# zbqq/neus2

Hardware: AMD Instinct MI355X
Metric: training samples/sec (compacted NeuS2 training samples, DTU-scan24-shaped synthetic, base.json) (higher is better)
Workload: dtype fp16 MFMA (fp32 accumulate) / fp32 optimizer; 1 GPU; NeuS2 train step, Config S, base.json L=14 T=2^19 W=64, Nc=2^18/GPU, R=2^18/GPU fixed, all 14 levels active (network trained 800 steps before the warm-up); global_batch=262144, rays_per_gpu=262144, parallelism=dp1, prepare_steps=800, levels_active=14

## Files before the change

include/neus2_hip.h:

```cpp
#ifndef NEUS2_HIP_H
#define NEUS2_HIP_H

#include <stdint.h>

#ifdef __cplusplus
extern "C" {
#endif

typedef struct NeusTestbed NeusTestbed;

typedef struct NeusNetworkConfig {
	uint32_t n_levels;
	uint32_t n_features_per_level;
	uint32_t log2_hashmap_size;
	uint32_t base_resolution;
	float per_level_scale;
	float top_resolution;
	float valid_level_scale;
	float base_valid_level_scale;
	uint32_t base_training_step;
	uint32_t n_neurons;
	uint32_t n_density_hidden;
	uint32_t n_rgb_hidden;
	float learning_rate, beta1, beta2, epsilon, l2_reg;
// ... 135 lines not shown
	float background_color[3];
	int32_t color_space;
	int32_t linear_colors;
	float cone_angle_constant;
	float near_distance;
	float depth_supervision_lambda;
} NeusTrainingOptions;
int neus_testbed_get_training_options(NeusTestbed* tb, NeusTrainingOptions* out);
typedef struct NeusOptimizerState {
	uint32_t n_params;
	uint32_t current_step;
	float learning_rate;
	float learning_rate_factor;
} NeusOptimizerState;
int neus_testbed_get_optimizer_state(NeusTestbed* tb, NeusOptimizerState* st, float* m1, float* m2, uint32_t* steps, uint16_t* ema_half);
int neus_testbed_set_optimizer_state(NeusTestbed* tb, const NeusOptimizerState* st, const float* m1, const float* m2, const uint32_t* steps,
                                     const uint16_t* ema_half);
int neus_testbed_set_training_options(NeusTestbed* tb, const NeusTrainingOptions* opts);
int neus_testbed_set_progressive_inference(NeusTestbed* tb, int mode, const uint32_t* chunk_ends, uint32_t n_ends);
int neus_testbed_ray_counts(NeusTestbed* tb, uint32_t n, uint32_t* nreq, uint32_t* ccount, uint32_t* numsteps );
int neus_debug_time_kernel(NeusTestbed* tb, int kernel, int variant, int iters, float* ms_out);
int neus_testbed_time_kernel(NeusTestbed* tb, int kernel, int iters, float* ms_out, uint32_t* units_out);
int neus_debug_march_stats(NeusTestbed* tb, uint32_t n, uint32_t* out);
int neus_debug_march_profile(NeusTestbed* tb, unsigned long long* out, uint32_t max_waves, uint32_t* n_waves);
int neus_debug_scatter_stats(NeusTestbed* tb, uint64_t* records_per_level, uint32_t* max_region);
int neus_debug_scatter_parts(NeusTestbed* tb, uint32_t* parts_per_level );
int neus_debug_grid_scatter(NeusTestbed* tb, void* hip_stream, uint32_t n_cap, const uint32_t* n_valid, const float* coords,
                            uint32_t coord_stride, uint32_t valid_level, const void* dLdenc, const void* genc, const float* v,
                            float* grid_grad_out);
int neus_debug_mlp_train(NeusTestbed* tb, void* hip_stream, uint32_t n, const float* coords, const uint16_t* enc, const float* dydx,
                         const uint16_t* dL_dout, uint32_t indeed_batch_size, float* grads_out, float* dpos, uint16_t* genc_out,
                         uint16_t* dLdenc_out, uint16_t* d1_delta_out, float* v_out);
int neus_debug_exclusive_scan(void* hip_stream, const uint32_t* in, uint32_t* out, uint32_t n, int reps, uint32_t* failures);
int neus_debug_scan_giveup(void* hip_stream, const uint32_t* in, uint32_t* out, uint32_t n, uint32_t* failures);
int neus_debug_inject_health(NeusTestbed* tb, uint32_t flags);
int neus_debug_set_lds_fill(NeusTestbed* tb, uint32_t pattern);
int neus_debug_set_lds_fill_all(NeusTestbed* tb, uint32_t pattern);
int neus_debug_set_xcd_shift(NeusTestbed* tb, uint32_t n_blocks);
int neus_debug_set_grid_generic(uint32_t on);
int neus_debug_get_batch(NeusTestbed* tb, float* coords_out, uint16_t* dl_dout_out, float* loss_out);
int neus_debug_denorm_probe(int device, uint32_t n, uint32_t launches, uint64_t* stats);
int neus_debug_get_buffer(NeusTestbed* tb, int id, uint64_t offset, uint64_t nbytes, void* host);
int neus_debug_replay_loss_grad(NeusTestbed* tb, uint16_t* dl_dout_out);
int neus_debug_sample_rays_round0(NeusTestbed* tb, void* stream, uint32_t n_rays, uint32_t n_rays_total, uint64_t rng_state, uint64_t rng_inc,
                                  uint32_t max_samples, const uint8_t* bitfield, float* rays, uint32_t* numsteps, float* coords,
                                  uint32_t* counters_out, uint32_t chunk_end, uint32_t* list, uint32_t* list_len, uint32_t lds_fill);
int neus_testbed_stream(NeusTestbed* tb, void** hip_stream);
int neus_testbed_synchronize(NeusTestbed* tb);
#define NEUS_N_PHASES 10
int neus_testbed_set_profiling(NeusTestbed* tb, int on);
int neus_testbed_kernel_times(NeusTestbed* tb, float* ms_out );
int neus_testbed_set_infer_timing(NeusTestbed* tb, int on);
int neus_testbed_infer_timing(NeusTestbed* tb, double* ms_total, uint64_t* launches, uint64_t* steps);
int neus_testbed_set_exchange_timing(NeusTestbed* tb, int on);
int neus_testbed_exchange_timing(NeusTestbed* tb, double* exposed_ms_total, double* span_ms_total, uint64_t* steps);

int neus_nccl_unique_id(uint8_t* out );
int neus_testbed_init_data_parallel(NeusTestbed* tb, int rank, int world, const uint8_t* unique_id );
#define NEUS_DP_FORCE_COLLECTIVES 1
int neus_testbed_init_data_parallel_ex(NeusTestbed* tb, int rank, int world, const uint8_t* unique_id, uint32_t flags);
typedef struct NeusDataParallelInfo {
	uint32_t rank, world;
	uint32_t has_communicator;
	uint32_t local_group;
	uint64_t collective_calls;
	uint64_t allreduce_bytes;
// ... 93 lines not shown
```

neus2_amd/_lib.py:

```python
from __future__ import annotations

import ctypes as C
import os

_HERE = os.path.dirname(os.path.abspath(__file__))
LIB_PATH = os.environ.get("NEUS2_HIP_LIB") or os.path.join(_HERE, "libneus2_hip.so")


class NeusNetworkConfig(C.Structure):
    _fields_ = [
        ("n_levels", C.c_uint32), ("n_features_per_level", C.c_uint32), ("log2_hashmap_size", C.c_uint32),
        ("base_resolution", C.c_uint32), ("per_level_scale", C.c_float), ("top_resolution", C.c_float),
        ("valid_level_scale", C.c_float), ("base_valid_level_scale", C.c_float), ("base_training_step", C.c_uint32),
        ("n_neurons", C.c_uint32), ("n_density_hidden", C.c_uint32), ("n_rgb_hidden", C.c_uint32),
        ("learning_rate", C.c_float), ("beta1", C.c_float), ("beta2", C.c_float), ("epsilon", C.c_float), ("l2_reg", C.c_float),
        ("ema_decay", C.c_float), ("decay_start", C.c_uint32), ("decay_interval", C.c_uint32), ("decay_base", C.c_float),
        ("ek_loss_weight", C.c_float), ("mask_loss_weight", C.c_float), ("anneal_end", C.c_uint32), ("batch_size", C.c_uint32),
        ("sdf_bias", C.c_float), ("density_grid_decay", C.c_float), ("seed", C.c_uint32), ("fixed_rays_per_batch", C.c_uint32),
        ("predict_global_movement", C.c_uint32), ("global_movement_steps", C.c_uint32), ("finetune_global_movement", C.c_uint32),
        ("reset_density_grid_after_global_movement", C.c_uint32), ("after_learning_rate", C.c_float),
        ("gm_learning_rate", C.c_float), ("gm_beta1", C.c_float), ("gm_beta2", C.c_float), ("gm_epsilon", C.c_float),
        ("gm_decay_start", C.c_uint32), ("gm_decay_interval", C.c_uint32), ("gm_decay_base", C.c_float),
    ]

# ... 50 lines not shown
        ("width", C.c_int32), ("height", C.c_int32), ("spp", C.c_uint32), ("training_view", C.c_int32),
        ("xform", C.c_float * 12), ("focal", C.c_float * 2), ("screen_center", C.c_float * 2),
        ("snap_to_pixel_centers", C.c_int32), ("min_transmittance", C.c_float), ("use_ema", C.c_int32),
    ]


class NeusTrainingOptions(C.Structure):
    _fields_ = [
        ("random_bg_color", C.c_int32), ("background_color", C.c_float * 3), ("color_space", C.c_int32),
        ("linear_colors", C.c_int32), ("cone_angle_constant", C.c_float), ("near_distance", C.c_float),
        ("depth_supervision_lambda", C.c_float),
    ]


class NeusOptimizerState(C.Structure):
    _fields_ = [("n_params", C.c_uint32), ("current_step", C.c_uint32), ("learning_rate", C.c_float),
                ("learning_rate_factor", C.c_float)]


class NeusModuleInfo(C.Structure):
    _fields_ = [("n_params", C.c_uint64), ("n_input_dims", C.c_uint32), ("n_output_dims", C.c_uint32),
                ("param_precision", C.c_int32), ("output_precision", C.c_int32), ("gradient_precision", C.c_int32),
                ("batch_capacity", C.c_uint32), ("n_levels", C.c_uint32), ("grid_offset", C.c_uint64),
                ("per_level_scale", C.c_float)]


EXPORTS = [
    "neus_last_error", "neus_abi_version", "neus_device_count", "neus_device_synchronize",
    "neus_testbed_create", "neus_testbed_destroy", "neus_testbed_set_dataset", "neus_testbed_reload_network",
    "neus_testbed_layout", "neus_testbed_train", "neus_testbed_get_stats", "neus_testbed_get_params",
    "neus_testbed_set_params", "neus_testbed_get_gradients", "neus_testbed_get_ema_params",
    "neus_testbed_get_half_params",
    "neus_testbed_get_density_grid", "neus_testbed_set_density_grid", "neus_testbed_restore_state", "neus_testbed_get_rng", "neus_testbed_render", "neus_testbed_sdf_on_grid",
    "neus_testbed_marching_cubes", "neus_testbed_mc_density", "neus_testbed_get_mesh", "neus_testbed_mesh_vertex_colors", "neus_mc_table", "neus_prepare_image_rgba8", "neus_testbed_ray_counts", "neus_debug_time_kernel", "neus_debug_march_stats", "neus_debug_exclusive_scan", "neus_debug_scan_giveup", "neus_debug_inject_health", "neus_debug_set_lds_fill", "neus_debug_set_lds_fill_all", "neus_debug_set_xcd_shift", "neus_debug_set_grid_generic", "neus_debug_denorm_probe", "neus_debug_get_batch", "neus_debug_get_buffer", "neus_debug_replay_loss_grad", "neus_debug_sample_rays_round0", "neus_debug_march_profile", "neus_debug_scatter_stats", "neus_debug_scatter_parts", "neus_debug_grid_scatter", "neus_debug_mlp_train", "neus_testbed_time_kernel", "neus_testbed_stream",
    "neus_testbed_synchronize", "neus_testbed_set_profiling", "neus_testbed_kernel_times", "neus_testbed_set_infer_timing", "neus_testbed_infer_timing",
    "neus_testbed_set_exchange_timing", "neus_testbed_exchange_timing",
    "neus_nccl_unique_id", "neus_testbed_init_data_parallel", "neus_testbed_init_data_parallel_ex",
    "neus_testbed_data_parallel_info", "neus_testbed_set_exchange_overlap", "neus_local_group_create", "neus_local_group_destroy",
    "neus_testbed_init_local_group", "neus_host_group_create", "neus_host_group_destroy", "neus_testbed_init_host_group", "neus_debug_host_group_allreduce",
    "neus_grid_encode", "neus_net_forward", "neus_net_backward", "neus_sample_rays", "neus_loss_compact",
    "neus_optimizer_step", "neus_fill_rollover", "neus_occ_update", "neus_mfma_probe",
    "neus_testbed_next_frame", "neus_testbed_get_movement", "neus_testbed_set_movement", "neus_testbed_frame_state",
    "neus_testbed_change_frame", "neus_testbed_prepare_for_test", "neus_testbed_get_training_options",
    "neus_testbed_set_training_options", "neus_testbed_saved_transform", "neus_testbed_get_optimizer_state",
    "neus_testbed_set_optimizer_state", "neus_testbed_set_progressive_inference",
    "neus_module_create_network", "neus_module_create_nerf_network", "neus_module_create_encoding", "neus_module_create_network_with_input_encoding", "neus_module_destroy", "neus_context_destroy",
    "neus_module_info", "neus_module_hyperparams", "neus_module_set_training_step", "neus_module_set_indeed_batch_size",
    "neus_module_initialize_params", "neus_module_inference", "neus_module_forward", "neus_module_backward",
    "neus_module_backward_backward_input",
    "neus_net_backward_pos", "neus_delta_apply", "neus_delta_backward",
    "neus_volrend_march_count", "neus_volrend_march_write", "neus_volrend_alpha_forward", "neus_volrend_alpha_backward",
    "neus_volrend_composite_forward", "neus_volrend_composite_backward",
]

ABI_VERSION = 9

_lib = None


def lib():
    global _lib
    if _lib is not None:
        return _lib
    if not os.path.exists(LIB_PATH):
        raise RuntimeError(f"{LIB_PATH} not found: build it with `python -c 'import __graft_entry__ as g; g.build()'`")
    l = C.CDLL(LIB_PATH)
    l.neus_last_error.restype = C.c_char_p
# ... 21 lines not shown
```

neus2_amd/csrc/kernels.h:

```cpp
#pragma once
#include <functional>
#include <vector>
#include "common.h"

namespace neus {

struct MlpPtrs {
	const half_t* d0;  const half_t* d1;
	const half_t* r0;  const half_t* r1;  const half_t* r2;
	const half_t* d0T; const half_t* d1T;
	const half_t* r0T; const half_t* r1T; const half_t* r2T;
	const half_t* d0p; const half_t* d0Tp;
	const half_t* var;
	float sdf_bias;
};

struct TrainBufs {
	half_t* d1_delta;
	half_t* dLdenc; half_t* genc;
	float4* v;
	float* var_grad;
	float* var_partial;
	float indeed_batch;
	float4* dpos;
// ... 242 lines not shown
uint32_t ray_sort_blocks(uint32_t cap);
void launch_ray_sort(hipStream_t s, uint32_t cap, const uint32_t* numsteps, const float* coords, uint32_t e1, const RaySort& rs, uint32_t* list,
                     uint32_t* list_len, void* scan_temp, size_t scan_temp_bytes, const RaySplit* split = nullptr);
void launch_march_write(hipStream_t s, uint32_t cap, StepState* st, const DevDataset& ds, const float* rays, const MarchWork& mw, const uint32_t* nreq,
                        uint32_t* base, uint32_t* numsteps, float* coords, uint32_t* sample_ray, uint32_t sample_cap, void* scan_temp,
                        const Round0List* round0 = nullptr, uint32_t lds_fill = 0 );
constexpr uint32_t FILL_LDS_BYTES = 40 * 1024;
void launch_fill_lds(hipStream_t s, uint32_t pattern);
extern thread_local uint32_t g_dbg_lds_fill;
extern thread_local uint32_t g_dbg_xcd_shift;
extern thread_local hipEvent_t g_infer_ev[2];
void debug_denorm_probe(hipStream_t s, uint32_t n, uint32_t launches, uint64_t* stats);
void launch_xcd_shift(hipStream_t s, uint32_t n_blocks);
inline void dbg_lds_gate(hipStream_t s) {
	if (g_dbg_lds_fill) launch_fill_lds(s, g_dbg_lds_fill);
	if (g_dbg_xcd_shift) launch_xcd_shift(s, g_dbg_xcd_shift);
}
void debug_launch_march_stats(hipStream_t s, uint32_t n_rays, const float* rays, const float* tstart, const uint32_t* lin, const DevDataset& ds,
                              const uint8_t* bf, uint32_t* out);
void launch_loss_alpha(hipStream_t s, uint32_t cap_samples, const StepState* st, const float* coords, const half_t* net_out, float cos_anneal,
                       const LossWork& w, bool dt_const = false);
void launch_loss_scan_ray(hipStream_t s, uint32_t cap_rays, const uint32_t* numsteps, const LossWork& w, uint32_t* ccount);
void launch_loss_alpha_list(hipStream_t s, uint32_t cap_samples, const uint32_t* n_ptr, const uint32_t* idx, const float* coords,
                            const half_t* net_out, float cos_anneal, const LossWork& w, bool dt_const = false);
void launch_prog_cut(hipStream_t s, uint32_t cap_rays, const uint32_t* ccount, const uint32_t* excl, uint32_t batch, uint32_t* cutw, int mode,
                     uint32_t* eval0, uint32_t* abort_if_none = nullptr);
void launch_scan_prog_cut(hipStream_t s, void* scan_temp, const uint32_t* ccount, uint32_t* excl, uint32_t n, uint32_t batch, uint32_t* cutw, int mode,
                          uint32_t* eval0, uint32_t* abort_if_none = nullptr);
void launch_prog_next(hipStream_t s, uint32_t cap_rays, const uint32_t* rays_in, const uint32_t* n_in, const uint32_t* numsteps, const uint32_t* cut,
                      uint32_t e1, uint32_t e2, uint32_t* list, uint32_t* list_counter, uint32_t* rays_out, uint32_t* n_out);
void launch_loss_scan_chunk(hipStream_t s, uint32_t cap_rays, const uint32_t* numsteps, const LossWork& w, uint32_t* ccount, uint32_t e0,
                            uint32_t e1, uint32_t e2, uint32_t* list , uint32_t* next_counter,
                            const uint32_t* rays_in = nullptr, const uint32_t* n_rays_in = nullptr, uint32_t* rays_out = nullptr,
                            uint32_t* n_rays_out = nullptr);
void launch_srgb_lut(hipStream_t s, float* lut);
void launch_loss_ray(hipStream_t s, uint32_t cap_rays, StepState* st, DPInfo dp, const DevDataset& ds, const LossParams& lp, uint32_t* numsteps,
                     const uint32_t* ccount, const uint32_t* cbase, const LossWork& w, float* loss, float* ek, float* mask);
void launch_loss_grad(hipStream_t s, uint32_t cap_samples, StepState* st, DPInfo dp, const LossParams& lp, const float* coords,
                      const half_t* net_out, const uint32_t* numsteps, const LossWork& w, float* coords_out, half_t* dL_dout);
void debug_launch_loss_scan(hipStream_t s, int variant, uint32_t cap_rays, const uint32_t* numsteps, const LossWork& w, uint32_t* ccount);
void launch_ray_index(hipStream_t s, uint32_t cap_rays, const uint32_t* numsteps, StepState* st, uint32_t* sample_ray, uint32_t* rbase);
void launch_rollover(hipStream_t s, uint32_t n_elements, const StepState* st, float* coords, half_t* dL_dout);
void launch_step_counters(hipStream_t s, StepState* st, uint32_t target_batch, uint32_t max_samples, uint32_t world, uint32_t fixed_rays,
                          const uint32_t* eval_cnt = nullptr, uint32_t n_eval = 0, uint32_t* abort_host = nullptr);
size_t render_ray_bytes();
void launch_render_init(hipStream_t s, const RenderCamera& cam, uint32_t sample_index, const DevDataset& ds, const uint8_t* bf, const uint32_t* lin,
                        void* rays, float4* frame);
void launch_render_compact(hipStream_t s, uint32_t n, const void* src, uint32_t* flags, uint32_t* base, void* dst, uint32_t* n_alive,
                           void* scan_tmp, size_t scan_tmp_bytes);
void launch_render_gen(hipStream_t s, uint32_t n_alive, uint32_t n_steps, const DevDataset& ds, const uint8_t* bf, const uint32_t* lin, void* rays,
                       float* coords);
void launch_render_composite(hipStream_t s, uint32_t n_alive, uint32_t n_steps, const float* coords, const half_t* net_out, float cos_anneal,
                             float min_transmittance, bool linear_colors, void* rays, float4* frame);
void launch_render_accumulate(hipStream_t s, uint32_t n, uint32_t spp, const float4* frame, float4* accum);
uint32_t mc_n_chunks(const uint32_t res[3]);
void mc_table_host(int8_t* out );
void launch_mc_count(hipStream_t s, const uint32_t res[3], const float amin[3], const float amax[3], float thresh, const float* density,
                     uint32_t* cnt_v, uint32_t* cnt_t);
void launch_mc_emit(hipStream_t s, const uint32_t res[3], const float amin[3], const float amax[3], float thresh, const float* density,
                    const uint32_t* off_v, const uint32_t* off_t, float* verts, uint32_t* vidx, uint32_t* tris);
void launch_mesh_coords(hipStream_t s, uint32_t n, const float* verts, const DevDataset& ds, float* coords);
void launch_mesh_unmove(hipStream_t s, uint32_t n, const RayMotion& m, float* verts);
void launch_delta_prepare(hipStream_t s, DeltaState* ds);
void launch_delta_apply(hipStream_t s, const uint32_t* n_ptr, uint32_t n_cap, uint32_t stride, const float* in, float* out, const DeltaState* ds);
void launch_delta_backward(hipStream_t s, const uint32_t* n_ptr, uint32_t n_cap, const float* coords, uint32_t stride, const float4* dpos,
                           DeltaState* ds, float* partial, const DeltaAdam& a);
void launch_delta_grad(hipStream_t s, const uint32_t* n_ptr, uint32_t n_cap, const float* coords, uint32_t stride, const float4* dpos,
// ... 86 lines not shown
```

neus2_amd/csrc/march.hip:

```cpp
#pragma clang fp contract(off)
#include "march_common.h"
#include "scan_lookback.h"
#include <algorithm>
#include <cstdlib>
#include <cstring>
#include <vector>

namespace neus {



__global__ void k_bitfield_linear(const uint8_t* __restrict__ bf, uint32_t* __restrict__ lin) {
	const uint32_t w = blockIdx.x * blockDim.x + threadIdx.x;
	if (w >= GRID3 / 32) return;
	const uint32_t ix = w >> 9, iy = (w >> 2) & 127, iz0 = (w & 3) * 32;
	uint32_t word = 0;
	for (uint32_t b = 0; b < 32; ++b) {
		const uint32_t idx = morton3D(ix, iy, iz0 + b);
		word |= (uint32_t)((bf[idx / 8] >> (idx % 8)) & 1) << b;
	}
	lin[w] = word;
}
__device__ __forceinline__ bool ray_hits_box(const float o[3], const float d[3], const float bb[6]) {
	float tn = 0.0f, tf = 3.402823466e+38f;
// ... 1120 lines not shown
			}
		}
		if (open) {
			ccount[i] = S.cn;
			racc[i] = make_float4(S.r0, S.r1, S.r2, S.ws);
			rT[i] = S.T;
			rek[i] = S.ek;
		}
		if (list || rays_out) {
			const uint32_t m = (open && S.cn == e1 && e1 < ns && S.T >= 1e-4f) ? min(ns, e2) - e1 : 0u;
			const uint32_t incl = wave_incl_sum(m);
			const uint32_t total = wave_lane_value(incl, 63);
			if (total) {
				if (list) {
					uint32_t p0 = 0;
					if (lane == 0) p0 = atomicAdd(next_counter, total);
					p0 = wave_lane_value(p0, 0);
					const uint32_t pre = incl - m, src = base + e1;
					unsigned long long todo = __ballot(m > 0);
					while (todo) {
						const int o = __ffsll(todo) - 1;
						todo &= todo - 1ull;
						const uint32_t m_o = wave_lane_value(m, o), p_o = p0 + wave_lane_value(pre, o), s_o = wave_lane_value(src, o);
						for (uint32_t j = lane; j < m_o; j += 64) list[p_o + j] = s_o + j;
					}
				}
				if (rays_out) {
					const unsigned long long mk = __ballot(m > 0);
					uint32_t q0 = 0;
					if (lane == 0) q0 = atomicAdd(n_rays_out, (uint32_t)__popcll(mk));
					q0 = wave_lane_value(q0, 0);
					if (m > 0) rays_out[q0 + (uint32_t)__popcll(mk & ((1ull << lane) - 1ull))] = i;
				}
			}
		}
	}
}

__global__ void __launch_bounds__(256) k_prog_cut(uint32_t cap_rays, const uint32_t* __restrict__ ccount, const uint32_t* __restrict__ excl,
                                                  uint32_t batch, uint32_t* __restrict__ cutw, int mode, uint32_t* __restrict__ eval0,
                                                  uint32_t* __restrict__ abort_if_none) {
	const uint32_t i = blockIdx.x * blockDim.x + threadIdx.x;
	if (i >= cap_rays) return;
	const uint32_t e = excl[i], incl = e + ccount[i];
	const bool cross = e < batch && incl >= batch, none = i == cap_rays - 1 && incl < batch;
	if (!cross && !none) return;
	const uint32_t c = cross ? i : cap_rays;
	if (mode == 0) {
		cutw[CW_CUT_A] = c;
		cutw[CW_LENB_EFF] = cross ? 0u : cutw[CW_LENB];
		cutw[CW_NB_EFF] = cross ? 0u : cutw[CW_NB];
	} else {
		cutw[CW_CUT] = c;
		cutw[CW_EST] = min(cap_rays, (c + c / 4u + 1024u + 63u) & ~63u);
		if (eval0) *eval0 += cutw[CW_LENB_EFF];
		if (abort_if_none && !cross) *abort_if_none = 1u;
	}
}
__global__ void __launch_bounds__(SCAN_THREADS) k_scan_prog_cut(const uint32_t* __restrict__ ccount, uint32_t* __restrict__ excl, uint32_t n,
                                                                ScanState* __restrict__ ss, uint32_t tag, uint32_t batch, uint32_t* __restrict__ cutw,
                                                                int mode, uint32_t* __restrict__ eval0, uint32_t* __restrict__ abort_if_none) {
	__shared__ uint32_t s_prefix, s_wsum[SCAN_THREADS / 64];
	const ScanTile tl = scan_tile(tag);
	const size_t b0 = (size_t)tl.tile * SCAN_TILE + (size_t)threadIdx.x * SCAN_ITEMS;
	uint32_t v[SCAN_ITEMS];
	scan_load16(ccount, b0, n, true, v);
// ... 397 lines not shown
void launch_march_write(hipStream_t s, uint32_t cap, StepState* st, const DevDataset& ds, const float* rays, const MarchWork& mw, const uint32_t* nreq,
                        uint32_t* base, uint32_t* numsteps, float* coords, uint32_t* sample_ray, uint32_t sample_cap, void* scan_temp,
                        const Round0List* round0, uint32_t lds_fill) {
	const Round0List r0 = round0 ? *round0 : Round0List{0u, nullptr, nullptr, nullptr, 0u};
	if (cap % 4 || ((uintptr_t)nreq | (uintptr_t)base | (uintptr_t)numsteps | (uintptr_t)r0.c0) & 15)
		throw std::runtime_error("launch_march_write: ray buffers must be 16-B aligned, cap a multiple of 4");
	const uint32_t tiles = (cap + SCAN_TILE - 1) / SCAN_TILE;
	if (tiles > SCAN_MAX_TILES) throw std::runtime_error("launch_march_write: too many ray slots");
	dbg_lds_gate(s);
	k_march_scan<<<tiles, SCAN_THREADS, 0, s>>>(cap, st, nreq, base, numsteps, (ScanState*)scan_temp, scan_next_tag(scan_temp), r0);
	if (lds_fill) launch_fill_lds(s, lds_fill);
	else dbg_lds_gate(s);
	k_march_write<<<std::max<uint32_t>(1, (sample_cap + WRITE_CHUNK - 1) / WRITE_CHUNK), 256, 0, s>>>(cap, st, ds, rays, mw, nreq, base, coords, sample_ray,
	                                                                                                      r0);
}
void debug_launch_march_stats(hipStream_t s, uint32_t n_rays, const float* rays, const float* tstart, const uint32_t* lin, const DevDataset& ds,
                              const uint8_t* bf, uint32_t* out) {
	k_march_stats<<<(n_rays + 255) / 256, 256, 0, s>>>(n_rays, rays, tstart, lin, ds, bf, out);
}
static inline uint32_t sample_blocks(uint32_t cap) { return std::max<uint32_t>(1, std::min<uint32_t>((cap + 255) / 256, 16384)); }
void launch_loss_alpha(hipStream_t s, uint32_t cap_samples, const StepState* st, const float* coords, const half_t* net_out, float cos_anneal,
                       const LossWork& w, bool dt_const) {
	dbg_lds_gate(s);
	k_loss_alpha<<<sample_blocks(cap_samples), 256, 0, s>>>(cap_samples, &st->n_kept, nullptr, coords, net_out, cos_anneal, w.sa, w.ekt, w.n_long,
	                                                        dt_const);
}
void launch_loss_alpha_list(hipStream_t s, uint32_t cap_samples, const uint32_t* n_ptr, const uint32_t* idx, const float* coords,
                            const half_t* net_out, float cos_anneal, const LossWork& w, bool dt_const) {
	dbg_lds_gate(s);
	k_loss_alpha<<<sample_blocks(cap_samples), 256, 0, s>>>(cap_samples, n_ptr, idx, coords, net_out, cos_anneal, w.sa, w.ekt, nullptr, dt_const);
}
void launch_loss_scan_chunk(hipStream_t s, uint32_t cap_rays, const uint32_t* numsteps, const LossWork& w, uint32_t* ccount, uint32_t e0,
                            uint32_t e1, uint32_t e2, uint32_t* list, uint32_t* next_counter, const uint32_t* rays_in, const uint32_t* n_rays_in,
                            uint32_t* rays_out, uint32_t* n_rays_out) {
	dbg_lds_gate(s);
	k_loss_scan_chunk<<<std::max<uint32_t>(1, std::min<uint32_t>((cap_rays + 63) / 64, 8192)), 64, 0, s>>>(
		cap_rays, numsteps, w.sa, w.ekt, w.ck4, w.cke, ccount, w.racc, w.rT, w.rek, e0, e1, e2, list, next_counter, rays_in, n_rays_in,
		rays_out, n_rays_out);
}
void launch_prog_cut(hipStream_t s, uint32_t cap_rays, const uint32_t* ccount, const uint32_t* excl, uint32_t batch, uint32_t* cutw, int mode,
                     uint32_t* eval0, uint32_t* abort_if_none) {
	k_prog_cut<<<(cap_rays + 255) / 256, 256, 0, s>>>(cap_rays, ccount, excl, batch, cutw, mode, eval0, abort_if_none);
}
void launch_prog_next(hipStream_t s, uint32_t cap_rays, const uint32_t* rays_in, const uint32_t* n_in, const uint32_t* numsteps, const uint32_t* cut,
                      uint32_t e1, uint32_t e2, uint32_t* list, uint32_t* list_counter, uint32_t* rays_out, uint32_t* n_out) {
	k_prog_next<<<std::max<uint32_t>(1, std::min<uint32_t>((cap_rays + 255) / 256, 1024)), 256, 0, s>>>(rays_in, n_in, numsteps, cut, e1, e2, list,
	                                                                                                   list_counter, rays_out, n_out);
}
void launch_loss_scan_ray(hipStream_t s, uint32_t cap_rays, const uint32_t* numsteps, const LossWork& w, uint32_t* ccount) {
	const uint32_t blocks = ray_blocks(cap_rays);
	dbg_lds_gate(s);
	k_loss_scan_ray<true><<<blocks, 256, 0, s>>>(cap_rays, numsteps, w.sa, w.ekt, w.ck4, w.cke, ccount, w.racc, w.rT, w.long_rays, w.n_long);
	if (w.long_rays) dbg_lds_gate(s);
	if (w.long_rays) k_loss_scan_list<<<std::max<uint32_t>(1, std::min<uint32_t>((cap_rays + 63) / 64, 4096)), 64, 0, s>>>(
		numsteps, w.sa, w.ekt, w.ck4, w.cke, ccount, w.racc, w.rT, w.long_rays, w.n_long);
}
void debug_launch_loss_scan(hipStream_t s, int variant, uint32_t cap_rays, const uint32_t* numsteps, const LossWork& w, uint32_t* ccount) {
	if (variant == 1) k_loss_scan_ray<false><<<ray_blocks(cap_rays), 256, 0, s>>>(cap_rays, numsteps, w.sa, w.ekt, w.ck4, w.cke, ccount, w.racc, w.rT,
	                                                                           nullptr, nullptr);
	else {
		if (w.n_long) (void)hipMemsetAsync(w.n_long, 0, 4, s);
		launch_loss_scan_ray(s, cap_rays, numsteps, w, ccount);
	}
}
__global__ void k_srgb_lut(float* __restrict__ lut) {
	const uint32_t b = threadIdx.x;
	lut[b] = srgb_to_linear((float)b * (1.0f / 255.0f));
}
// ... 29 lines not shown
```

neus2_amd/csrc/options.h:

```cpp
#pragma once

#include <algorithm>
#include <cstdint>
#include <cstdio>
#include <cstdlib>
#include <cstring>
#include <vector>

namespace neus_env {
inline bool on_unless_0(const char* name) { const char* e = std::getenv(name); return !(e && e[0] == '0'); }
inline bool off_unless_1(const char* name) { const char* e = std::getenv(name); return e && e[0] == '1'; }
inline bool is(const char* name, const char* value) { const char* e = std::getenv(name); return e && std::strcmp(e, value) == 0; }
inline int as_int(const char* name, int def) { const char* e = std::getenv(name); return e ? std::atoi(e) : def; }
inline uint32_t as_u32(const char* name, uint32_t def) { const char* e = std::getenv(name); return e ? (uint32_t)std::strtoul(e, nullptr, 10) : def; }
inline float as_float(const char* name, float def) { const char* e = std::getenv(name); return e ? (float)std::atof(e) : def; }
inline std::vector<uint32_t> increasing_list(const char* name) {
	std::vector<uint32_t> v;
	const char* e = std::getenv(name);
	if (!e) return v;
	for (const char* p = e; *p;) { char* q = nullptr; const unsigned long x = std::strtoul(p, &q, 10); if (q == p) break; v.push_back((uint32_t)x); p = *q ? q + 1 : q; }
	bool ok = !v.empty() && v.size() <= 14 && v[0] > 0;
	for (size_t k = 1; k < v.size(); ++k) ok = ok && v[k] > v[k - 1];
	if (!ok) v.clear();
	return v;
}
}

struct NeusOptions {
	bool main_prio = true;
	bool lookahead = true;
	int la_at_cut = 1;
	int la_at_full = 0;
	int la_prio = -1;
	bool ev_sysfence = false;
	bool la_stat = false;
	bool adam_overlap = false;
	bool exchange_overlap = true;
	bool eager_ema_h = false;

	uint32_t march_waves = 0;
	uint32_t march_lanes = 8;
	bool march_balance = true;
	uint32_t march_dbg = 0;
	bool ray_cull = true;
	bool ray_sort = true;
	bool prog_cut = true;
	bool march_cut = true;
	uint32_t march_cut_div = 1;
	std::vector<uint32_t> chunk_ends;
	float chunk_scale = 2.f;
	int chunk_rounds = 2;

	bool occ_sort = true;
	bool occ_nu_sort = false;

	uint32_t scatter_mode = 2;
	uint32_t scatter_chunk = 512;
	uint32_t scatter_level_groups = 0;
	uint32_t scatter_xcd_group = 4;
	bool scatter_noskip = false;

	bool dbg_loss_replay = false;
	bool dbg_loss_fence = false;

	static NeusOptions from_env() {
		using namespace neus_env;
		NeusOptions o;
		o.main_prio = on_unless_0("NEUS_MAIN_PRIO");
		o.lookahead = on_unless_0("NEUS_LOOKAHEAD");
		o.la_at_cut = as_int("NEUS_LA_AT", o.la_at_cut);
		o.la_at_full = as_int("NEUS_LA_AT_FULL", o.la_at_full);
		o.la_prio = as_int("NEUS_LA_PRIO", o.la_prio);
		o.ev_sysfence = off_unless_1("NEUS_EV_SYSFENCE");
		o.la_stat = off_unless_1("NEUS_LA_STAT");
		o.adam_overlap = off_unless_1("NEUS_ADAM_OVERLAP");
		o.exchange_overlap = on_unless_0("NEUS_EXCHANGE_OVERLAP");
		o.eager_ema_h = off_unless_1("NEUS_EAGER_EMA_H");
		o.march_waves = as_u32("NEUS_MARCH_WAVES", o.march_waves);
		{ const uint32_t v = as_u32("NEUS_MARCH_LANES", 8); o.march_lanes = v == 1 || v == 4 || v == 16 ? v : 8u; }
		o.march_balance = on_unless_0("NEUS_MARCH_BALANCE");
		o.march_dbg = as_u32("NEUS_MARCH_DBG", o.march_dbg);
		o.ray_cull = on_unless_0("NEUS_RAY_CULL");
		o.ray_sort = on_unless_0("NEUS_RAY_SORT");
		o.prog_cut = on_unless_0("NEUS_PROG_CUT");
		o.march_cut = on_unless_0("NEUS_MARCH_CUT");
		o.march_cut_div = (uint32_t)std::max(1, as_int("NEUS_DBG_MARCH_CUT_DIV", 1));
		o.chunk_ends = increasing_list("NEUS_CHUNK_ENDS");
		o.chunk_scale = as_float("NEUS_CHUNK_SCALE", o.chunk_scale);
		o.chunk_rounds = as_int("NEUS_CHUNK_ROUNDS", o.chunk_rounds);
		o.occ_sort = on_unless_0("NEUS_OCC_SORT");
		o.occ_nu_sort = off_unless_1("NEUS_OCC_NU_SORT");
		o.scatter_mode = is("NEUS_SCATTER", "binned") ? 1u : is("NEUS_SCATTER", "wide") ? 0u : 2u;
		o.scatter_chunk = is("NEUS_SCATTER_CHUNK", "1024") ? 1024u : is("NEUS_SCATTER_CHUNK", "256") ? 256u : 512u;
		if (o.scatter_mode != 2 && o.scatter_chunk == 256) o.scatter_chunk = 512;
		o.scatter_level_groups = (uint32_t)std::max(0, as_int("NEUS_SCATTER_LG", 0));
		o.scatter_xcd_group = std::max(1u, as_u32("NEUS_SC_XCD_GROUP", o.scatter_xcd_group));
		o.scatter_noskip = off_unless_1("NEUS_SCATTER_NOSKIP");
		o.dbg_loss_replay = off_unless_1("NEUS_DBG_LOSS_REPLAY");
		o.dbg_loss_fence = off_unless_1("NEUS_DBG_LOSS_FENCE");
		return o;
	}
};

struct NeusProcessOptions {
	bool infer_xcd_parts = false;
	bool infer_pipe = true;
	uint32_t infer_grid = 0;
	uint32_t mlp_blocks_pct = 100;
	static NeusProcessOptions from_env() {
		using namespace neus_env;
		NeusProcessOptions o;
		o.infer_xcd_parts = off_unless_1("NEUS_INFER_XCD_PARTS");
		o.infer_pipe = on_unless_0("NEUS_INFER_PIPE");
		o.infer_grid = (uint32_t)as_int("NEUS_INFER_GRID", 0);
		o.mlp_blocks_pct = (uint32_t)as_int("NEUS_MLP_BLOCKS_PCT", 100);
		return o;
	}
};
inline const NeusProcessOptions& process_options() {
	static const NeusProcessOptions o = NeusProcessOptions::from_env();
	return o;
}
// ... 14 lines not shown
```

neus2_amd/csrc/testbed.cpp:

```cpp
#include <rocprofiler-sdk-roctx/roctx.h>
#include "kernels.h"
#include "scan_lookback.h"
#include "json_lite.h"
#include "hostgroup.h"
#include "options.h"
#include "host_util.h"
#include "core.h"
#include "../../include/neus2_hip.h"

#include <rccl/rccl.h>

#include <algorithm>
#include <atomic>
#include <cstdio>
#include <functional>
#include <chrono>
#include <cmath>
#include <condition_variable>
#include <mutex>
#include <cstdlib>
#include <cstring>
#include <memory>
#include <random>
#include <stdexcept>
// ... 1383 lines not shown
		const bool sorted_rays = progressive && opt.ray_sort;
		const RaySort rsort{rs_hist.p, rs_off.p, rs_key.p, rs_perm.p, chunk_cnt.p + RS_N_PERM};
		if (la_have) {
			if (canonical_step % n_prep == 0) throw std::runtime_error("train: lookahead issued before an occupancy update");
			++la_steps;
			if (opt.la_stat && la_stat_used % 4 == 2) HIP_CHECK(hipEventRecord(la_stat_next(), s));
			HIP_CHECK(hipStreamWaitEvent(s, ev_la_done.get(), 0));
			if (opt.la_stat && la_stat_used % 4 == 3) HIP_CHECK(hipEventRecord(la_stat_next(), s));
		}
		const bool cut = la_have ? la_cut : cut_for(training_step, progressive, call_left == 0, dyn);
		const std::vector<uint32_t>& ce = ends_for(cut);
		const uint32_t nch = (uint32_t)ce.size() + 1;
		const bool mcut = la_have ? la_mcut : march_cut_for(training_step, cut && sorted_rays, call_left);
		if (!la_have) issue_march(s, dp, rng, progressive, scan_tmp.p, cut, mcut);
		mc_hist[0] = mcut;
		const bool risky = (mc_hist[0] || mc_hist[1]) && !force_full;
		const bool split = cut && sorted_rays;
		if (cut) ++cut_steps;
		if (mcut) ++mcut_steps;
		mark(2);
		const float* c_in = coords.p;
		if (use_delta) { launch_delta_apply(s, &st.p->n_kept, max_samples, COORD_W, coords.p, coords_def.p, delta.p); c_in = coords_def.p; }
		LossParams lp{};
		lp.loss_scale = LOSS_SCALE; lp.ek_w = cfg.ek_loss_weight; lp.mask_w = cfg.mask_loss_weight; lp.cos_anneal = cos_anneal();
		lp.max_compacted = batch; lp.rng_state = rng.state; lp.rng_inc = rng.inc; lp.jt = jump_table();
		lp.abort_w = cutw.p + CW_ABORT; lp.abort_slot = training_step & 1u;
		if (risky && !coll_on()) {
			lp.abort_host = arm_abort_word();
		}
		lp.dbg_fence = opt.dbg_loss_fence ? 1u : 0u;
		const LossWork w = loss_work(base.p);
		if (progressive) {
			uint32_t e0 = 0;
			for (uint32_t k = 0; k < nch; ++k) {
				const uint32_t e1 = k + 1 < nch ? ce[k] : 0xffffffffu;
				const uint32_t e2 = k + 2 < nch ? ce[k + 1] : 0xffffffffu;
				const InferAlpha ia{w.sa, w.ekt, lp.cos_anneal, ds.cone_angle == 0.0f ? 1u : 0u, nullptr, sorted_rays ? 8u : 0u};
				it_arm();
				launch_nerf_infer(s, lay.L, lay.W, chunk_cnt.p + k, 0, c_in, gl, valid, params_h.p + lay.grid_off, mlp, net_out.p, 8192, chunk_list.p,
				                  use_delta ? nullptr : &ia);
				if (use_delta) launch_loss_alpha_list(s, max_samples, chunk_cnt.p + k, chunk_list.p, coords.p, net_out.p, lp.cos_anneal, w, ds.cone_angle == 0.0f);
				const bool more = k + 1 < nch;
				const bool cut_k = cut && k == 0 && more;
				launch_loss_scan_chunk(s, MAX_RAYS, numsteps.p, w, ccount.p, e0, e1, e2, more && !cut_k ? chunk_list.p : nullptr, chunk_cnt.p + k + 1,
				                       k ? open_rays[(k - 1) & 1].p : (sorted_rays ? rs_perm.p : nullptr),
				                       k ? chunk_cnt.p + OPEN_CNT + k - 1 : (sorted_rays ? rsort.n_perm : nullptr),
				                       more ? (cut_k ? open_raw.p : open_rays[k & 1].p) : nullptr,
				                       more ? chunk_cnt.p + (cut_k ? RAW_CNT : OPEN_CNT) + k : nullptr);
				if (cut_k) {
					const bool split_b = split && !mcut;
					if (split_b) {
						launch_scan_prog_cut(s, scan_tmp.p, ccount.p, cbase.p, MAX_RAYS, batch, cutw.p, 0, nullptr);
						const InferAlpha iab{w.sa, w.ekt, lp.cos_anneal, ds.cone_angle == 0.0f ? 1u : 0u, nullptr, 8u};
						it_arm();
						launch_nerf_infer(s, lay.L, lay.W, cutw.p + CW_LENB_EFF, 0, c_in, gl, valid, params_h.p + lay.grid_off, mlp, net_out.p, 8192,
						                  chunk_list.p + max_samples, &iab);
						launch_loss_scan_chunk(s, MAX_RAYS, numsteps.p, w, ccount.p, 0, e1, e2, nullptr, nullptr, rs_perm.p + MAX_RAYS,
						                       cutw.p + CW_NB_EFF, open_raw.p, chunk_cnt.p + RAW_CNT + k);
					}
					launch_scan_prog_cut(s, scan_tmp.p, ccount.p, cbase.p, MAX_RAYS, batch, cutw.p, 1, split_b ? chunk_cnt.p : nullptr,
					                     mcut ? cutw.p + CW_ABORT + (training_step & 1u) : nullptr);
					launch_prog_next(s, MAX_RAYS, open_raw.p, chunk_cnt.p + RAW_CNT + k, numsteps.p, cutw.p + CW_CUT, e1, e2, chunk_list.p,
					                 chunk_cnt.p + k + 1, open_rays[k & 1].p, chunk_cnt.p + OPEN_CNT + k);
				}
				e0 = e1;
			}
			mark(3);
		} else {
			const InferAlpha ia{w.sa, w.ekt, lp.cos_anneal, ds.cone_angle == 0.0f ? 1u : 0u, w.n_long};
			it_arm();
			launch_nerf_infer(s, lay.L, lay.W, &st.p->n_kept, 0, c_in, gl, valid, params_h.p + lay.grid_off, mlp, net_out.p, 8192, nullptr,
			                  use_delta ? nullptr : &ia);
			mark(3);
			if (use_delta) launch_loss_alpha(s, max_samples, st.p, coords.p, net_out.p, lp.cos_anneal, w, ds.cone_angle == 0.0f);
			launch_loss_scan_ray(s, MAX_RAYS, numsteps.p, w, ccount.p);
		}
		launch_exclusive_scan(s, scan_tmp.p, scan_tmp_bytes, ccount.p, cbase.p, MAX_RAYS);
		launch_loss_ray(s, MAX_RAYS, st.p, dp, ds, lp, numsteps.p, ccount.p, cbase.p, w, loss.p, ek.p, mask.p);
		launch_loss_grad(s, max_samples, st.p, dp, lp, coords.p, net_out.p, numsteps.p, w, coords_c.p, dL_dout.p);
		if (opt.dbg_loss_replay) {
			dbg_co.alloc((size_t)batch * COORD_W); dbg_dl.alloc((size_t)batch * OUT_W);
			launch_loss_grad(s, max_samples, st.p, dp, lp, coords.p, net_out.p, numsteps.p, w, dbg_co.p, dbg_dl.p);
			const std::pair<const void*, size_t> src[DBG_SNAP_N] = {
				{l_sa.p, l_sa.n * 16}, {l_ekt.p, l_ekt.n * 4}, {l_ck4.p, l_ck4.n * 16}, {l_cke.p, l_cke.n * 4}, {l_racc.p, l_racc.n * 16},
				{l_rgr.p, l_rgr.n * 16}, {l_rT.p, l_rT.n * 4}, {l_rek.p, l_rek.n * 4}, {ccount.p, ccount.n * 4}, {net_out.p, net_out.n * 2},
				{coords.p, coords.n * 4}, {base.p, base.n * 4}, {numsteps.p, numsteps.n * 4}, {cmap.p, cmap.n * 4}, {nreq.p, nreq.n * 4}};
			for (int k = 0; k < DBG_SNAP_N; ++k) {
				dbg_snap[k].alloc(src[k].second);
				HIP_CHECK(hipMemcpyAsync(dbg_snap[k].p, src[k].first, src[k].second, hipMemcpyDeviceToDevice, s));
			}
		}
// ... 887 lines not shown
		if (v_out) HIP_CHECK(hipMemcpyAsync(v_out, t.v, (size_t)n * sizeof(float4), hipMemcpyDeviceToDevice, s));
		HIP_CHECK(hipStreamSynchronize(s));
	});
}
int neus_debug_march_profile(NeusTestbed* tb, unsigned long long* out, uint32_t max_waves, uint32_t* n_waves) {
	return guard([&] {
		if (!tb->have_net) throw std::runtime_error("no network");
		NeusTestbed& t = *tb;
		hipStream_t s = t.stream;
		const uint32_t waves = MAX_RAYS * t.mwork.lanes_per_ray / 64;
		Dev<unsigned long long> buf; buf.alloc((size_t)waves * 8);
		HIP_CHECK(hipMemsetAsync(buf.p, 0, (size_t)waves * 64, s));
		MarchWork mw = t.mwork;
		mw.prof = buf.p;
		mw.dbg = t.opt.march_dbg;
		launch_march_count(s, MAX_RAYS, t.max_samples, t.st.p, DPInfo{t.rank, t.world}, t.ds, t.bitfield.p, t.bf_lin.p, t.rng.state, t.rng.inc,
		                   t.rays.p, t.startt.p, t.nreq.p, mw, nullptr, 0, t.opt.ray_cull ? t.occ_bbox.p : nullptr);
		HIP_CHECK(hipStreamSynchronize(s));
		const uint32_t n = std::min(waves, max_waves);
		HIP_CHECK(hipMemcpy(out, buf.p, (size_t)n * 64, hipMemcpyDeviceToHost));
		if (n_waves) *n_waves = n;
	});
}
int neus_debug_exclusive_scan(void* stream, const uint32_t* in, uint32_t* out, uint32_t n, int reps, uint32_t* failures) {
	return guard([&] {
		hipStream_t s = (hipStream_t)stream;
		const size_t tb_ = scan_temp_bytes(std::max(1u, n));
		ScanTemp tmp; tmp.alloc(tb_ + 256); scan_temp_reset(s, tmp.p);
		for (int r = 0; r < std::max(1, reps); ++r) launch_exclusive_scan(s, tmp.p, tb_, in, out, n);
		HIP_CHECK(hipStreamSynchronize(s));
		if (failures) *failures = scan_failures(tmp.p);
	});
}
int neus_testbed_stream(NeusTestbed* tb, void** s) { return guard([&] { *s = (void*)tb->stream; }); }
int neus_testbed_synchronize(NeusTestbed* tb) { return guard([&] { HIP_CHECK(hipStreamSynchronize(tb->stream)); }); }
int neus_testbed_set_profiling(NeusTestbed* tb, int on) {
	return guard([&] {
		tb->flush_phases();
		tb->profiling = on != 0;
		for (auto& m : tb->phase_ms) m = 0;
		tb->phase_steps = 0; tb->phase_npre = tb->phase_ntrain = 0;
	});
}
int neus_testbed_set_infer_timing(NeusTestbed* tb, int on) {
	return guard([&] {
		tb->infer_timing = on != 0;
		tb->it_n = 0; tb->it_ms = 0.0; tb->it_launches = 0; tb->it_steps = 0;
	});
}
int neus_testbed_infer_timing(NeusTestbed* tb, double* ms_total, uint64_t* launches, uint64_t* steps) {
	return guard([&] {
		if (ms_total) *ms_total = tb->it_ms;
		if (launches) *launches = tb->it_launches;
		if (steps) *steps = tb->it_steps;
	});
}
int neus_testbed_set_exchange_timing(NeusTestbed* tb, int on) {
	return guard([&] {
		tb->xt_collect_all();
		tb->xt_on = on != 0;
		tb->xt_exposed_ms = tb->xt_span_ms = 0.0; tb->xt_steps = 0;
	});
}
int neus_testbed_exchange_timing(NeusTestbed* tb, double* exposed_ms_total, double* span_ms_total, uint64_t* steps) {
	return guard([&] {
		HIP_CHECK(hipSetDevice(tb->device));
// ... 410 lines not shown
```

Before: 343.2 million samples/s.

## Add 16-lane-per-ray grouped loss scan kernel for progressive chunk scans

Adds a new loss-scan kernel that assigns each ray to a 16-lane DPP row and computes transmittance and color accumulation as a parallel prefix scan across the row, instead of one lane walking each ray serially. It prefetches several 16-sample slices ahead, uses ballots to find the early-termination point, and appends next-chunk sample lists per block with a single atomic. It is enabled by default when the cut path is active, or forced through NEUS_SCAN_FORM. The aim is to shorten the serial per-ray dependency chain and coalesce sample loads, at the cost of more DPP/permute work and wasted lanes on short rays.

```diff
diff --git a/include/neus2_hip.h b/include/neus2_hip.h
--- a/include/neus2_hip.h
+++ b/include/neus2_hip.h
@@ -191,6 +191,10 @@
                          const uint16_t* dL_dout, uint32_t indeed_batch_size, float* grads_out, float* dpos, uint16_t* genc_out,
                          uint16_t* dLdenc_out, uint16_t* d1_delta_out, float* v_out);
 int neus_debug_exclusive_scan(void* hip_stream, const uint32_t* in, uint32_t* out, uint32_t n, int reps, uint32_t* failures);
+int neus_debug_loss_scan_chunk(void* hip_stream, int form, uint32_t n_rays, const uint32_t* numsteps, const float* sa, const float* ekt,
+                               uint32_t e0, uint32_t e1, uint32_t e2, const uint32_t* rays_in, const uint32_t* n_rays_in, uint32_t* ccount,
+                               float* racc, float* rT, float* rek, float* ck4, float* cke, uint32_t* list, uint32_t* list_counter,
+                               uint32_t* rays_out, uint32_t* rays_out_counter);
 int neus_debug_scan_giveup(void* hip_stream, const uint32_t* in, uint32_t* out, uint32_t n, uint32_t* failures);
 int neus_debug_inject_health(NeusTestbed* tb, uint32_t flags);
 int neus_debug_set_lds_fill(NeusTestbed* tb, uint32_t pattern);
diff --git a/neus2_amd/_lib.py b/neus2_amd/_lib.py
--- a/neus2_amd/_lib.py
+++ b/neus2_amd/_lib.py
@@ -106,7 +106,7 @@
     "neus_testbed_set_params", "neus_testbed_get_gradients", "neus_testbed_get_ema_params",
     "neus_testbed_get_half_params",
     "neus_testbed_get_density_grid", "neus_testbed_set_density_grid", "neus_testbed_restore_state", "neus_testbed_get_rng", "neus_testbed_render", "neus_testbed_sdf_on_grid",
-    "neus_testbed_marching_cubes", "neus_testbed_mc_density", "neus_testbed_get_mesh", "neus_testbed_mesh_vertex_colors", "neus_mc_table", "neus_prepare_image_rgba8", "neus_testbed_ray_counts", "neus_debug_time_kernel", "neus_debug_march_stats", "neus_debug_exclusive_scan", "neus_debug_scan_giveup", "neus_debug_inject_health", "neus_debug_set_lds_fill", "neus_debug_set_lds_fill_all", "neus_debug_set_xcd_shift", "neus_debug_set_grid_generic", "neus_debug_denorm_probe", "neus_debug_get_batch", "neus_debug_get_buffer", "neus_debug_replay_loss_grad", "neus_debug_sample_rays_round0", "neus_debug_march_profile", "neus_debug_scatter_stats", "neus_debug_scatter_parts", "neus_debug_grid_scatter", "neus_debug_mlp_train", "neus_testbed_time_kernel", "neus_testbed_stream",
+    "neus_testbed_marching_cubes", "neus_testbed_mc_density", "neus_testbed_get_mesh", "neus_testbed_mesh_vertex_colors", "neus_mc_table", "neus_prepare_image_rgba8", "neus_testbed_ray_counts", "neus_debug_time_kernel", "neus_debug_march_stats", "neus_debug_exclusive_scan", "neus_debug_loss_scan_chunk","neus_debug_scan_giveup", "neus_debug_inject_health", "neus_debug_set_lds_fill", "neus_debug_set_lds_fill_all", "neus_debug_set_xcd_shift", "neus_debug_set_grid_generic", "neus_debug_denorm_probe", "neus_debug_get_batch", "neus_debug_get_buffer", "neus_debug_replay_loss_grad", "neus_debug_sample_rays_round0", "neus_debug_march_profile", "neus_debug_scatter_stats", "neus_debug_scatter_parts", "neus_debug_grid_scatter", "neus_debug_mlp_train", "neus_testbed_time_kernel", "neus_testbed_stream",
     "neus_testbed_synchronize", "neus_testbed_set_profiling", "neus_testbed_kernel_times", "neus_testbed_set_infer_timing", "neus_testbed_infer_timing",
     "neus_testbed_set_exchange_timing", "neus_testbed_exchange_timing",
     "neus_nccl_unique_id", "neus_testbed_init_data_parallel", "neus_testbed_init_data_parallel_ex",
diff --git a/neus2_amd/csrc/kernels.h b/neus2_amd/csrc/kernels.h
--- a/neus2_amd/csrc/kernels.h
+++ b/neus2_amd/csrc/kernels.h
@@ -298,7 +298,7 @@
 void launch_loss_scan_chunk(hipStream_t s, uint32_t cap_rays, const uint32_t* numsteps, const LossWork& w, uint32_t* ccount, uint32_t e0,
                             uint32_t e1, uint32_t e2, uint32_t* list , uint32_t* next_counter,
                             const uint32_t* rays_in = nullptr, const uint32_t* n_rays_in = nullptr, uint32_t* rays_out = nullptr,
-                            uint32_t* n_rays_out = nullptr);
+                            uint32_t* n_rays_out = nullptr, bool group = false);
 void launch_srgb_lut(hipStream_t s, float* lut);
 void launch_loss_ray(hipStream_t s, uint32_t cap_rays, StepState* st, DPInfo dp, const DevDataset& ds, const LossParams& lp, uint32_t* numsteps,
                      const uint32_t* ccount, const uint32_t* cbase, const LossWork& w, float* loss, float* ek, float* mask);
diff --git a/neus2_amd/csrc/march.hip b/neus2_amd/csrc/march.hip
--- a/neus2_amd/csrc/march.hip
+++ b/neus2_amd/csrc/march.hip
@@ -1176,6 +1176,126 @@
 					q0 = wave_lane_value(q0, 0);
 					if (m > 0) rays_out[q0 + (uint32_t)__popcll(mk & ((1ull << lane) - 1ull))] = i;
 				}
+			}
+		}
+	}
+}
+
+constexpr uint32_t SCAN_G = 16;
+__device__ __forceinline__ float row_prev(float carry, float x) { return dpp_f32<DPP_ROW_SHR + 1>(carry, x); }
+__device__ __forceinline__ float row_prev0(float x) {
+	return __builtin_bit_cast(float, __builtin_amdgcn_update_dpp(0, __builtin_bit_cast(int, x), DPP_ROW_SHR + 1, 0xf, 0xf, true));
+}
+__device__ __forceinline__ float lane_get(float x, uint32_t src_lane) {
+	return __builtin_bit_cast(float, __builtin_amdgcn_ds_bpermute((int)(src_lane << 2), __builtin_bit_cast(int, x)));
+}
+__global__ void __launch_bounds__(256) k_loss_scan_chunk_group(uint32_t cap_rays, const uint32_t* __restrict__ numsteps, const float4* __restrict__ sa,
+                                                               const float* __restrict__ ekt, float4* __restrict__ ck4, float* __restrict__ cke,
+                                                               uint32_t* __restrict__ ccount, float4* __restrict__ racc, float* __restrict__ rT,
+                                                               float* __restrict__ rek, uint32_t e0, uint32_t e1, uint32_t e2,
+                                                               uint32_t* __restrict__ list, uint32_t* __restrict__ next_counter,
+                                                               const uint32_t* __restrict__ rays_in, const uint32_t* __restrict__ n_rays_in,
+                                                               uint32_t* __restrict__ rays_out, uint32_t* __restrict__ n_rays_out) {
+	constexpr uint32_t G = SCAN_G, RPB = 256 / G, NB = 4;
+	static_assert(G == 16, "a ray's lanes are one DPP row");
+	typedef float f4v __attribute__((ext_vector_type(4)));
+	__shared__ uint32_t s_app[3 * RPB + 2];
+	const uint32_t tid = threadIdx.x, row = tid / G, el = tid % G, row0 = tid & 48u;
+	const char* sab = (const char*)sa;
+	const char* ekb = (const char*)ekt;
+	const uint32_t n_slots = rays_in ? min(*n_rays_in, cap_rays) : cap_rays;
+	for (uint32_t w0 = blockIdx.x * RPB; w0 < n_slots; w0 += gridDim.x * RPB) {
+		const bool inr = w0 + row < n_slots;
+		const uint32_t i = rays_in ? (inr ? rays_in[w0 + row] : 0u) : w0 + row;
+		const uint32_t ns = inr ? numsteps[2 * i] : 0u, base = inr ? numsteps[2 * i + 1] : 0u;
+		RayScan S{1.f, 0.f, 0.f, 0.f, 0.f, 0.f, 0u};
+		bool open = inr && (e0 == 0 || ns > 0);
+		if (e0 > 0 && inr) {
+			const uint32_t cn = ccount[i];
+			const float T = rT[i];
+			const float4 a = racc[i];
+			const float ek = rek[i];
+			S.cn = cn;
+			if (!open || cn != e0 || e0 >= ns || T < 1e-4f) open = false;
+			else { S.T = T; S.r0 = a.x; S.r1 = a.y; S.r2 = a.z; S.ws = a.w; S.ek = ek; }
+		}
+		const uint32_t to = min(ns, e1);
+		bool live = open && to > e0;
+		const uint32_t g0 = live ? base + e0 : 0u, gl = live ? base + to - 1u : 0u;
+		auto fetch = [&](f4v& q, float& e, uint32_t c) {
+			const uint32_t g = min(g0 + c + el, gl);
+			q = *(const f4v*)(sab + ((size_t)g << 4));
+			e = *(const float*)(ekb + ((size_t)g << 2));
+		};
+		auto slice = [&](f4v& qs, float& es, uint32_t c) {
+			const f4v q = qs; const float e = es;
+			fetch(qs, es, c + NB * G);
+			const float f = 1.f - q[0];
+			float t = S.T, P = S.T;
+#pragma unroll
+			for (uint32_t u = 0; u < G; ++u) { t = row_prev(S.T, P); P = t * f; }
+			const bool ok = (e0 + c + el < to) && !(t < 1e-4f);
+			const uint32_t stop = (uint32_t)(~__ballot(ok) >> row0) & 0xffffu;
+			const uint32_t nlive = live ? (stop ? (uint32_t)__ffs(stop) - 1u : G) : 0u;
+			const float w = q[0] * t;
+			const float p0 = w * q[1], p1 = w * q[2], p2 = w * q[3];
+			const bool first = el == 0;
+			const float v0 = first ? S.r0 + p0 : p0, v1 = first ? S.r1 + p1 : p1, v2 = first ? S.r2 + p2 : p2;
+			const float vw = first ? S.ws + w : w, ve = first ? S.ek + e : e;
+			float a0 = v0, a1 = v1, a2 = v2, aw = vw, ae = ve;
+#pragma unroll
+			for (uint32_t u = 1; u < G; ++u) {
+				a0 = row_prev0(a0) + v0; a1 = row_prev0(a1) + v1; a2 = row_prev0(a2) + v2; aw = row_prev0(aw) + vw; ae = row_prev0(ae) + ve;
+			}
+			const float b0 = row_prev(S.r0, a0), b1 = row_prev(S.r1, a1), b2 = row_prev(S.r2, a2), be = row_prev(S.ek, ae);
+			const uint32_t s = base + e0 + c + el;
+			if (el < nlive && (s & (SCAN_CK - 1)) == 0) { ck4[s / SCAN_CK] = make_float4(t, b0, b1, b2); cke[s / SCAN_CK] = be; }
+			const uint32_t src = row0 + (nlive ? nlive - 1u : 0u);
+			const float nT = lane_get(P, src), n0 = lane_get(a0, src), n1 = lane_get(a1, src), n2 = lane_get(a2, src);
+			const float nw = lane_get(aw, src), ne = lane_get(ae, src);
+			if (nlive) { S.T = nT; S.r0 = n0; S.r1 = n1; S.r2 = n2; S.ws = nw; S.ek = ne; }
+			S.cn += nlive;
+			live = nlive == G;
+		};
+		if (__ballot(live)) {
+			f4v qs[NB]; float es[NB];
+#pragma unroll
+			for (uint32_t bf = 0; bf < NB; ++bf) fetch(qs[bf], es[bf], bf * G);
+			for (uint32_t c = 0;; c += NB * G) {
+				bool more = true;
+#pragma unroll
+				for (uint32_t bf = 0; bf < NB; ++bf) {
+					if (more && __ballot(live && e0 + c + bf * G < to) == 0) more = false;
+					if (more) slice(qs[bf], es[bf], c + bf * G);
+				}
+				if (!more) break;
+			}
+		}
+		if (open && el == 0) {
+			ccount[i] = S.cn;
+			racc[i] = make_float4(S.r0, S.r1, S.r2, S.ws);
+			rT[i] = S.T;
+			rek[i] = S.ek;
+		}
+		if (list || rays_out) {
+			const uint32_t m = (open && S.cn == e1 && e1 < ns && S.T >= 1e-4f) ? min(ns, e2) - e1 : 0u;
+			__syncthreads();
+			if (el == 0) { s_app[row] = m; s_app[RPB + row] = base + e1; s_app[2 * RPB + row] = i; }
+			__syncthreads();
+			if (tid == 0) {
+				uint32_t total = 0, n_open = 0;
+				for (uint32_t r = 0; r < RPB; ++r) { total += s_app[r]; n_open += s_app[r] ? 1u : 0u; }
+				s_app[3 * RPB] = list && total ? atomicAdd(next_counter, total) : 0u;
+				s_app[3 * RPB + 1] = rays_out && total ? atomicAdd(n_rays_out, n_open) : 0u;
+			}
+			__syncthreads();
+			uint32_t p = s_app[3 * RPB], k = s_app[3 * RPB + 1];
+			for (uint32_t r = 0; r < RPB; ++r) {
+				const uint32_t m_r = s_app[r];
+				if (m_r == 0) continue;
+				if (list) { const uint32_t s_r = s_app[RPB + r]; for (uint32_t j = tid; j < m_r; j += 256) list[p + j] = s_r + j; }
+				if (rays_out && tid == r) rays_out[k] = s_app[2 * RPB + r];
+				p += m_r; ++k;
 			}
 		}
 	}
@@ -1639,8 +1759,14 @@
 }
 void launch_loss_scan_chunk(hipStream_t s, uint32_t cap_rays, const uint32_t* numsteps, const LossWork& w, uint32_t* ccount, uint32_t e0,
                             uint32_t e1, uint32_t e2, uint32_t* list, uint32_t* next_counter, const uint32_t* rays_in, const uint32_t* n_rays_in,
-                            uint32_t* rays_out, uint32_t* n_rays_out) {
+                            uint32_t* rays_out, uint32_t* n_rays_out, bool group) {
 	dbg_lds_gate(s);
+	if (group) {
+		k_loss_scan_chunk_group<<<std::max<uint32_t>(1, std::min<uint32_t>((cap_rays + 15) / 16, 2048)), 256, 0, s>>>(
+			cap_rays, numsteps, w.sa, w.ekt, w.ck4, w.cke, ccount, w.racc, w.rT, w.rek, e0, e1, e2, list, next_counter, rays_in, n_rays_in,
+			rays_out, n_rays_out);
+		return;
+	}
 	k_loss_scan_chunk<<<std::max<uint32_t>(1, std::min<uint32_t>((cap_rays + 63) / 64, 8192)), 64, 0, s>>>(
 		cap_rays, numsteps, w.sa, w.ekt, w.ck4, w.cke, ccount, w.racc, w.rT, w.rek, e0, e1, e2, list, next_counter, rays_in, n_rays_in,
 		rays_out, n_rays_out);
diff --git a/neus2_amd/csrc/options.h b/neus2_amd/csrc/options.h
--- a/neus2_amd/csrc/options.h
+++ b/neus2_amd/csrc/options.h
@@ -50,6 +50,7 @@
 	std::vector<uint32_t> chunk_ends;
 	float chunk_scale = 2.f;
 	int chunk_rounds = 2;
+	uint32_t scan_form = 0;
 
 	bool occ_sort = true;
 	bool occ_nu_sort = false;
@@ -88,6 +89,7 @@
 		o.chunk_ends = increasing_list("NEUS_CHUNK_ENDS");
 		o.chunk_scale = as_float("NEUS_CHUNK_SCALE", o.chunk_scale);
 		o.chunk_rounds = as_int("NEUS_CHUNK_ROUNDS", o.chunk_rounds);
+		o.scan_form = is("NEUS_SCAN_FORM", "lane") ? 1u : is("NEUS_SCAN_FORM", "group") ? 2u : 0u;
 		o.occ_sort = on_unless_0("NEUS_OCC_SORT");
 		o.occ_nu_sort = off_unless_1("NEUS_OCC_NU_SORT");
 		o.scatter_mode = is("NEUS_SCATTER", "binned") ? 1u : is("NEUS_SCATTER", "wide") ? 0u : 2u;
diff --git a/neus2_amd/csrc/testbed.cpp b/neus2_amd/csrc/testbed.cpp
--- a/neus2_amd/csrc/testbed.cpp
+++ b/neus2_amd/csrc/testbed.cpp
@@ -1439,6 +1439,7 @@
 		const LossWork w = loss_work(base.p);
 		if (progressive) {
 			uint32_t e0 = 0;
+			const bool scan_group = opt.scan_form == 2 || (opt.scan_form == 0 && cut);
 			for (uint32_t k = 0; k < nch; ++k) {
 				const uint32_t e1 = k + 1 < nch ? ce[k] : 0xffffffffu;
 				const uint32_t e2 = k + 2 < nch ? ce[k + 1] : 0xffffffffu;
@@ -1453,7 +1454,7 @@
 				                       k ? open_rays[(k - 1) & 1].p : (sorted_rays ? rs_perm.p : nullptr),
 				                       k ? chunk_cnt.p + OPEN_CNT + k - 1 : (sorted_rays ? rsort.n_perm : nullptr),
 				                       more ? (cut_k ? open_raw.p : open_rays[k & 1].p) : nullptr,
-				                       more ? chunk_cnt.p + (cut_k ? RAW_CNT : OPEN_CNT) + k : nullptr);
+				                       more ? chunk_cnt.p + (cut_k ? RAW_CNT : OPEN_CNT) + k : nullptr, scan_group);
 				if (cut_k) {
 					const bool split_b = split && !mcut;
 					if (split_b) {
@@ -1463,7 +1464,7 @@
 						launch_nerf_infer(s, lay.L, lay.W, cutw.p + CW_LENB_EFF, 0, c_in, gl, valid, params_h.p + lay.grid_off, mlp, net_out.p, 8192,
 						                  chunk_list.p + max_samples, &iab);
 						launch_loss_scan_chunk(s, MAX_RAYS, numsteps.p, w, ccount.p, 0, e1, e2, nullptr, nullptr, rs_perm.p + MAX_RAYS,
-						                       cutw.p + CW_NB_EFF, open_raw.p, chunk_cnt.p + RAW_CNT + k);
+						                       cutw.p + CW_NB_EFF, open_raw.p, chunk_cnt.p + RAW_CNT + k, scan_group);
 					}
 					launch_scan_prog_cut(s, scan_tmp.p, ccount.p, cbase.p, MAX_RAYS, batch, cutw.p, 1, split_b ? chunk_cnt.p : nullptr,
 					                     mcut ? cutw.p + CW_ABORT + (training_step & 1u) : nullptr);
@@ -2417,6 +2418,23 @@
 		if (failures) *failures = scan_failures(tmp.p);
 	});
 }
+int neus_debug_loss_scan_chunk(void* stream, int form, uint32_t n_rays, const uint32_t* numsteps, const float* sa, const float* ekt, uint32_t e0,
+                               uint32_t e1, uint32_t e2, const uint32_t* rays_in, const uint32_t* n_rays_in, uint32_t* ccount, float* racc, float* rT,
+                               float* rek, float* ck4, float* cke, uint32_t* list, uint32_t* list_counter, uint32_t* rays_out,
+                               uint32_t* rays_out_counter) {
+	return guard([&] {
+		if (form != 0 && form != 1) throw std::runtime_error("neus_debug_loss_scan_chunk: form is 0 (lane) or 1 (group)");
+		if ((rays_in != nullptr) != (n_rays_in != nullptr) || (list && !list_counter) || (rays_out && !rays_out_counter))
+			throw std::runtime_error("neus_debug_loss_scan_chunk: a list without its counter");
+		hipStream_t s = (hipStream_t)stream;
+		LossWork w{};
+		w.sa = (float4*)sa; w.ekt = (float*)ekt; w.ck4 = (float4*)ck4; w.cke = cke; w.racc = (float4*)racc; w.rT = rT; w.rek = rek;
+		launch_loss_scan_chunk(s, n_rays, numsteps, w, ccount, e0, e1, e2, list, list_counter, rays_in, n_rays_in, rays_out, rays_out_counter,
+		                       form == 1);
+		HIP_CHECK(hipGetLastError());
+		HIP_CHECK(hipStreamSynchronize(s));
+	});
+}
 int neus_testbed_stream(NeusTestbed* tb, void** s) { return guard([&] { *s = (void*)tb->stream; }); }
 int neus_testbed_synchronize(NeusTestbed* tb) { return guard([&] { HIP_CHECK(hipStreamSynchronize(tb->stream)); }); }
 int neus_testbed_set_profiling(NeusTestbed* tb, int on) {
```

Result: faster. 350.4 million samples/s, median of 6 (+2.1%).
